# sergree/matchering

Hardware: NVIDIA H100
Metric: stereo 44.1kHz samples/sec (x real-time) (higher is better)
Workload: dtype f32

## Files before the change

### matchering_b200/csrc/common.cuh

```cuda
#pragma once

#ifndef MGB_EMULATE
#include <cuda_runtime.h>
#endif
#include <stdint.h>

#include "../../include/matchering_b200.h"

namespace mgb {

void set_error(const char* fmt, ...);
int cuda_status(const char* what);

#define MGB_REQUIRE(cond, code, ...)     \
    do {                                 \
        if (!(cond)) {                   \
            ::mgb::set_error(__VA_ARGS__); \
            return (code);               \
        }                                \
    } while (0)

#define MGB_TRY(expr)                 \
    do {                              \
        int mgb_rc_ = (expr);         \
        if (mgb_rc_ != MGB_OK) return mgb_rc_; \
    } while (0)

#ifdef MGB_EMULATE
#define MGB_DYN_SMEM(name) unsigned char* name = ::emul::dyn_smem()
template <typename... KA, typename... A>
inline int launch(const char* what, void (*kernel)(KA...), dim3 grid, dim3 block, size_t smem, cudaStream_t,
                  A... args) {
    (void)what;
    if (grid.x == 0 || grid.y == 0 || grid.z == 0) return MGB_OK;
    ::emul::launch(grid, block, smem, [&]() { kernel(static_cast<KA>(args)...); });
    return MGB_OK;
}
#else
#define MGB_DYN_SMEM(name) extern __shared__ __align__(128) unsigned char name[]
extern long long g_launch_count;
extern int g_profile;
void profile_mark(const char* what, cudaStream_t stream, bool begin);

template <typename... KA, typename... A>
inline int launch(const char* what, void (*kernel)(KA...), dim3 grid, dim3 block, size_t smem, cudaStream_t stream,
                  A... args) {
    if (grid.x == 0 || grid.y == 0 || grid.z == 0) return MGB_OK;
    g_launch_count++;
    if (smem > 48 * 1024) {
        static thread_local const void* done_kernel = nullptr;
        static thread_local size_t done_smem = 0;
        if (done_kernel != (const void*)kernel || done_smem < smem) {
            cudaError_t e = cudaFuncSetAttribute((const void*)kernel, cudaFuncAttributeMaxDynamicSharedMemorySize, (int)smem);
            if (e != cudaSuccess) {
                set_error("%s: cudaFuncSetAttribute(%zu B smem): %s", what, smem, cudaGetErrorString(e));
                return MGB_ERR_CUDA;
            }
            done_kernel = (const void*)kernel;
            done_smem = smem;
        }
    }
    if (g_profile) profile_mark(what, stream, true);
    kernel<<<grid, block, smem, stream>>>(static_cast<KA>(args)...);
    if (g_profile) profile_mark(what, stream, false);
    return cuda_status(what);
}
#endif

int num_sms();

template <typename T>
struct cpx {
    T x, y;
};
template <typename T>
__device__ __forceinline__ cpx<T> cmul(cpx<T> a, cpx<T> b) {
    return cpx<T>{a.x * b.x - a.y * b.y, a.x * b.y + a.y * b.x};
}
template <typename T>
__device__ __forceinline__ cpx<T> cadd(cpx<T> a, cpx<T> b) { return cpx<T>{a.x + b.x, a.y + b.y}; }
template <typename T>
__device__ __forceinline__ cpx<T> csub(cpx<T> a, cpx<T> b) { return cpx<T>{a.x - b.x, a.y - b.y}; }

__device__ __forceinline__ double warp_sum(double v) {
#pragma unroll
    for (int o = 16; o > 0; o >>= 1) v += __shfl_xor_sync(0xffffffffu, v, o);
    return v;
}
__device__ __forceinline__ float warp_max(float v) {
#pragma unroll
    for (int o = 16; o > 0; o >>= 1) v = fmaxf(v, __shfl_xor_sync(0xffffffffu, v, o));
    return v;
}

__device__ __forceinline__ double block_sum(double v, double* scratch) {
    const int lane = threadIdx.x & 31, warp = threadIdx.x >> 5, nwarps = (blockDim.x + 31) >> 5;
    v = warp_sum(v);
    __syncthreads();
    if (lane == 0) scratch[warp] = v;
    __syncthreads();
    if (warp == 0) {
        double t = (lane < nwarps) ? scratch[lane] : 0.0;
        t = warp_sum(t);
        if (lane == 0) scratch[0] = t;
    }
    __syncthreads();
    return scratch[0];
}
__device__ __forceinline__ float block_max(float v, float* scratch) {
    const int lane = threadIdx.x & 31, warp = threadIdx.x >> 5, nwarps = (blockDim.x + 31) >> 5;
    v = warp_max(v);
    __syncthreads();
    if (lane == 0) scratch[warp] = v;
    __syncthreads();
    if (warp == 0) {
        float t = (lane < nwarps) ? scratch[lane] : 0.0f;
        t = warp_max(t);
        if (lane == 0) scratch[0] = t;
    }
    __syncthreads();
    return scratch[0];
}

__device__ __forceinline__ unsigned warp_max_bits(unsigned v) {
#ifdef MGB_EMULATE
#pragma unroll
    for (int o = 16; o > 0; o >>= 1) {
        const unsigned other = __shfl_xor_sync(0xffffffffu, v, o);
        v = other > v ? other : v;
    }
    return v;
#else
    return __reduce_max_sync(0xffffffffu, v);
#endif
}
__device__ __forceinline__ void block_max2(float& a, float& b, unsigned* slot) {
    const unsigned ua = warp_max_bits(__float_as_uint(a)), ub = warp_max_bits(__float_as_uint(b));
    if ((threadIdx.x & 31) == 0) {
        atomicMax(&slot[0], ua);
        atomicMax(&slot[1], ub);
    }
    __syncthreads();
    a = __uint_as_float(slot[0]);
    b = __uint_as_float(slot[1]);
}

__device__ __forceinline__ float balance_factor(float large, float small) {
    if (!(small > 0.0f) || !(large > 0.0f)) return 1.0f;
    int e = (int)((__float_as_uint(large) >> 23) & 0xffu) - (int)((__float_as_uint(small) >> 23) & 0xffu);
    e = e < -60 ? -60 : (e > 60 ? 60 : e);
    return __uint_as_float((unsigned)(127 + e) << 23);
}

__device__ __forceinline__ float sqrt_approx(float x) {
#ifdef MGB_EMULATE
    return sqrtf(x);
#else
    float r;
    asm("sqrt.approx.ftz.f32 %0, %1;" : "=f"(r) : "f"(x));
    return r;
#endif
}

__device__ __forceinline__ void atomic_max_nonneg(float* addr, float v) {
    atomicMax(reinterpret_cast<int*>(addr), __float_as_int(v));
}
// ... 53 lines not shown
```

### matchering_b200/csrc/design.cu

```cuda
#include "fft.cuh"
#include "kernels.cuh"
#include "tail.cuh"

namespace mgb {

namespace {

constexpr int kDesignThreads = 512;
constexpr int kWarm = 48;
constexpr int kBatch = 16;
constexpr int kDesignBlocks = 4;

struct SplineTables {
    const double* hinv;
    const double* lu;
    const double* end;
};

__device__ void spline_moments(const double* __restrict__ y, int n, SplineTables t, double* __restrict__ z,
                               double* __restrict__ M) {
    const int m = n - 2;
    const double* fa = t.lu;
    const double* invden = t.lu + m;
    const double* cp = t.lu + 2 * m;
// ... 183 lines not shown
    double* M1 = m + HB;
    double* s = M1 + HB;
    double* mlog = s + HB;
    double* slog = mlog + NL;
    double* zz = slog + NL;
    double* M2 = zz + NL;

    spline_moments(m, HB, SplineTables{plan.d_sa_hinv, plan.d_sa_lu, plan.d_sa_end}, zz, M1);
    for (int j = tid; j < NL; j += nthr) mlog[j] = spline_eval(m, M1, plan.d_sa_eval_idx[j], plan.d_sa_eval_w + 4LL * j);
    __syncthreads();

    if (plan.lowess_it == 0) {
        const int k = plan.lowess_k;
        const int nfit = plan.lowess_nfit;
        for (int f = warp; f < nfit; f += 2 * nwarps) {
            const int f2 = min(f + nwarps, nfit - 1);
            const double* row_a = plan.d_lw_rows + (long long)plan.d_lw_row_idx[f] * k;
            const double* row_b = plan.d_lw_rows + (long long)plan.d_lw_row_idx[f2] * k;
            const double* ya = mlog + plan.d_lw_fit_left[f];
            const double* yb = mlog + plan.d_lw_fit_left[f2];
            double acc_a = 0.0, acc_b = 0.0;
            for (int j = lane; j < k; j += 32) {
                acc_a += row_a[j] * ya[j];
                acc_b += row_b[j] * yb[j];
            }
            acc_a = warp_sum(acc_a);
            acc_b = warp_sum(acc_b);
            if (lane == 0) {
                zz[f] = acc_a;
                zz[f2] = acc_b;
            }
        }
        __syncthreads();
        lowess_interpolate(plan, zz, slog);
    } else {
        double* resid_w = M2;
        for (int j = tid; j < NL; j += nthr) resid_w[j] = 1.0;
        __syncthreads();
        for (int pass = 0; pass <= plan.lowess_it; ++pass) {
            lowess_weighted_fits(plan, mlog, resid_w, zz);
            __syncthreads();
            lowess_interpolate(plan, zz, slog);
            if (pass < plan.lowess_it) lowess_residual_weights(mlog, slog, NL, zz, resid_w);
        }
    }

    spline_moments(slog, NL, SplineTables{plan.d_sb_hinv, plan.d_sb_lu, plan.d_sb_end}, zz, M2);
    for (int k = tid; k < HB; k += nthr) {
        double v = spline_eval(slog, M2, plan.d_sb_eval_idx[k], plan.d_sb_eval_w + 4LL * k);
        if (k == 0) v = 0.0;
        if (k == 1) v = m[1];
        s[k] = v;
    }
    __syncthreads();

}

struct DesignArgs {
    const float* spec_part_t;
    const float* spec_part_r;
    unsigned char* mask_t;
    unsigned char* mask_r;
    const float* absmax_t;
    float* target_peak;
    LevelsArgs levels;
    int div_t, slots_t, div_r, slots_r;
    long long frames_per_piece_t, frames_per_piece_r;
    const double* avg_override;
    double* scratch;
    long long stride;
    double* fir_out;
    float2* h_mid;
    float2* h_side;
    mgb_track_state* state;
    int s_ready;
    int ovs;
};

struct PrefetchList {
    const void* ptr[14];
    long long bytes[14];
    int count;
};

__device__ __forceinline__ void prefetch_l2(const void* p) {
#ifndef MGB_EMULATE
    asm volatile("prefetch.global.L2 [%0];" ::"l"(p));
#else
    (void)p;
#endif
}

constexpr int kMeanBins = 32, kMeanSlices = 32;

__global__ void __launch_bounds__(kMeanBins * kMeanSlices)
spectrum_mean_kernel(DesignArgs a, int n_lin, int fft_size, double eps, PrefetchList pf) {
    constexpr int BINS = kMeanBins, SLICES = kMeanSlices;
    __shared__ double part_t[SLICES][BINS + 1], part_r[SLICES][BINS + 1];
    MGB_DYN_SMEM(smem);
    unsigned char* mask_t = smem;
    unsigned char* mask_r = smem + a.div_t;
    {
        const long long gtid = ((long long)blockIdx.y * gridDim.x + blockIdx.x) * blockDim.x + threadIdx.x;
        const long long gsize = (long long)gridDim.x * gridDim.y * blockDim.x;
        for (int t = 0; t < pf.count; ++t)
            for (long long off = gtid * 128; off < pf.bytes[t]; off += gsize * 128)
                prefetch_l2(reinterpret_cast<const char*>(pf.ptr[t]) + off);
    }
    __shared__ LevelsResult lv_s;
    __shared__ unsigned peak_bits_s, target_peak_bits_s;
    double* piece_sum = reinterpret_cast<double*>(smem + ((a.div_t + a.div_r + 15) / 16) * 16);
    {
        const int lane = threadIdx.x & 31, warp = threadIdx.x >> 5, nwarps = blockDim.x >> 5;
        if (threadIdx.x == 0) peak_bits_s = target_peak_bits_s = 0u;
        __syncthreads();
        float pk = 0.0f;
        for (int i = threadIdx.x; i < a.div_r * a.slots_r + 1; i += blockDim.x) pk = fmaxf(pk, a.levels.absmax_r[i]);
        pk = warp_max_f(pk);
        if (lane == 0 && pk > 0.0f) atomicMax(&peak_bits_s, __float_as_uint(pk));
        if (blockIdx.x == 0 && blockIdx.y == 0) {
            float tpk = 0.0f;
            for (int i = threadIdx.x; i < a.div_t * a.slots_t + 1; i += blockDim.x) tpk = fmaxf(tpk, a.absmax_t[i]);
            tpk = warp_max_f(tpk);
            if (lane == 0 && tpk > 0.0f) atomicMax(&target_peak_bits_s, __float_as_uint(tpk));
        }
        for (int p = warp; p < a.div_t + a.div_r; p += nwarps) {
            const bool is_t = p < a.div_t;
            const double* part = is_t ? a.levels.sumsq_t + (long long)p * a.slots_t
                                      : a.levels.sumsq_r + (long long)(p - a.div_t) * a.slots_r;
            const int slots = is_t ? a.slots_t : a.slots_r;
            double sum = 0.0;
            for (int k = lane; k < slots; k += 32) sum += part[k];
            sum = warp_sum(sum);
            if (lane == 0) piece_sum[p] = sum;
        }
        __syncthreads();
        if (threadIdx.x < 32) {
            LevelsArgs folded = a.levels;
            folded.sumsq_t = piece_sum;
            folded.sumsq_r = piece_sum + a.div_t;
            folded.slots_t = folded.slots_r = 1;
            const float peak = __uint_as_float(peak_bits_s);
            folded.absmax_r = &peak;
            folded.div_r_items_override = 1;
            const LevelsResult mine = levels_compute_warp(folded, mask_t, mask_r);
            if (threadIdx.x == 0) lv_s = mine;
        }
    }
    __syncthreads();
    const LevelsResult lv = lv_s;
    if (blockIdx.x == 0 && blockIdx.y == 0) {
        if (threadIdx.x == 0) {
            levels_store(lv, a.state);
            a.state->conv_peak_bits = 0.0f;
            a.state->fir_peak_mid_bits = 0.0f;
            a.state->fir_peak_side_bits = 0.0f;
            a.state->conv_precise = 0;
            *a.target_peak = __uint_as_float(target_peak_bits_s);
        }
        for (int p = threadIdx.x; p < a.div_t; p += blockDim.x) a.mask_t[p] = mask_t[p];
        for (int p = threadIdx.x; p < a.div_r; p += blockDim.x) a.mask_r[p] = mask_r[p];
    }
    unsigned short* sel = reinterpret_cast<unsigned short*>(piece_sum + a.div_t + a.div_r);
    __shared__ int n_sel_s[2];
    int* piece_rank = reinterpret_cast<int*>(piece_sum);
    if (threadIdx.x < 32) {
        const int lane = threadIdx.x;
        for (int sig = 0; sig < 2; ++sig) {
            const unsigned char* mask = sig == 0 ? mask_t : mask_r;
            const int div = sig == 0 ? a.div_t : a.div_r;
            int* rank = piece_rank + (sig == 0 ? 0 : a.div_t);
            int count = 0;
            for (int base_p = 0; base_p < div; base_p += 32) {
                const int p = base_p + lane;
// ... 366 lines not shown
```

### matchering_b200/csrc/limiter.cu

```cuda
#include <math.h>
#include <string.h>

#include "limiter_scan.cuh"
#include "limiter_wide.cuh"

namespace mgb {

namespace {

constexpr int SPAN_EPT_MAX = kLimiterSpanEptMax;

__device__ __forceinline__ double scan_carry(double B, const ScanPow* t, double c0, double* scratch) {
    const int lane = threadIdx.x & 31, warp = threadIdx.x >> 5;
    double v = B;
#pragma unroll
    for (int d = 1; d < 32; d <<= 1) {
        const double up = __shfl_up_sync(0xffffffffu, v, d);
        if (lane >= d) v += t->ql[d] * up;
    }
    if (lane == 31) scratch[warp] = v;
    __syncthreads();
    double w = lane < NT / 32 ? scratch[lane] : 0.0;
#pragma unroll
    for (int d = 1; d < NT / 32; d <<= 1) {
        const double up = __shfl_up_sync(0xffffffffu, w, d);
        if (lane >= d) w += t->qw[d] * up;
    }
    const double warp_carry = __shfl_sync(0xffffffffu, w, (warp + 31) & 31);
    double prev = __shfl_up_sync(0xffffffffu, v, 1);
    if (lane == 0) prev = 0.0;
    return prev + t->ql[lane] * ((warp > 0 ? warp_carry : 0.0) + t->qw[warp] * c0);
}

__device__ __forceinline__ double scan_carry_rev(double B, const ScanPow* t, const double* c0, double* scratch) {
    const int lane = threadIdx.x & 31, warp = threadIdx.x >> 5;
    const int rl = 31 - lane, rw = NT / 32 - 1 - warp;
    double v = B;
#pragma unroll
    for (int d = 1; d < 32; d <<= 1) {
        const double up = __shfl_down_sync(0xffffffffu, v, d);
        if (rl >= d) v += t->ql[d] * up;
    }
    if (lane == 0) scratch[rw] = v;
    __syncthreads();
    double w = lane < NT / 32 ? scratch[lane] : 0.0;
#pragma unroll
    for (int d = 1; d < NT / 32; d <<= 1) {
        const double up = __shfl_up_sync(0xffffffffu, w, d);
        if (lane >= d) w += t->qw[d] * up;
    }
    const double warp_carry = __shfl_sync(0xffffffffu, w, (rw + 31) & 31);
    double prev = __shfl_down_sync(0xffffffffu, v, 1);
    if (rl == 0) prev = 0.0;
    return prev + t->ql[rl] * ((rw > 0 ? warp_carry : 0.0) + t->qw[rw] * (*c0));
}

struct LimiterGeom {
    int reach, hold, warm, left;
    int ept;
    int span;
    int filt;
    int publish_inclusive;
    int shared_core;
    int margin;
    int use_ticket;
};

__global__ void limiter_tables_kernel(mgb_limiter_params lp, int span_ept, unsigned char* tables) {
    const int i = threadIdx.x;
    ScanPow* att = reinterpret_cast<ScanPow*>(tables);
    {
        const double p = lp.attack_c;
        if (i < SPAN_EPT_MAX + 2) att->pe[i] = pow(p, (double)i);
        if (i < 33) att->ql[i] = pow(p, (double)(span_ept * i));
        if (i < 17) att->qw[i] = pow(p, (double)(span_ept * 32 * i));
        if (i < 33) att->pc[i] = pow(p, (double)LC * (double)i);
    }
    SectionTab<1>* sec = reinterpret_cast<SectionTab<1>*>(tables + sizeof(ScanPow));
    for (int f = 0; f < 2; ++f) {
        const double p = f == 0 ? -lp.hold_a[1] : -lp.release_a[1];
        SectionTab<1>* t = sec + f;
        if (i < CORE_EPT) t->pe[i][0] = pow(p, (double)(i + 1));
        if (i < 33) t->ql[i][0][0] = pow(p, (double)(CORE_EPT * i));
        if (i < 17) t->qw[i][0][0] = pow(p, (double)(CORE_EPT * 32 * i));
        if (i < 33) t->pc[i][0][0] = pow(p, (double)LC * (double)i);
        for (int j = i; j < kLookbackJumps; j += blockDim.x) t->pj[j][0][0] = pow(p, (double)LC * 32.0 * (double)j);
    }
}

template <int EPT, int NO, bool GAINS = false>
__global__ void __launch_bounds__(NT, (NO == 1 && EPT <= 17) ? 2 : 1)
limiter_kernel(mgb_limiter_params lp, LimiterGeom gm, const float2* __restrict__ in, float2* __restrict__ out,
               long long frames, const double* __restrict__ pre_gain, const double* __restrict__ post_gain,
               const int* __restrict__ engaged, int* __restrict__ ticket, LookbackWord* __restrict__ slots,
               const unsigned char* __restrict__ tables) {
    constexpr int HC = CORE_EPT + NO;
    constexpr int CAP = EPT * NT;
    MGB_DYN_SMEM(smem);
    double* Fd = reinterpret_cast<double*>(smem);
    float* Aenv = reinterpret_cast<float*>(smem) + CAP;
    float* G = reinterpret_cast<float*>(smem + (size_t)CAP * 8) + gm.margin;
    float* Wk = G + CAP + gm.margin;
    __shared__ float blockmax[NT];
    __shared__ ScanPow pw_att;
    __shared__ SectionTab<1> pw_sec[2];
    __shared__ double scratch_a[32 * NO], scratch_b[32 * NO];
    __shared__ double bcast[2 + 2 * NO];
    __shared__ int chunk_s;
    const ScanPow* pow_att = &pw_att;
    const SectionTab<NO>* sec_global = reinterpret_cast<const SectionTab<NO>*>(tables + sizeof(ScanPow));
    const SectionTab<NO>* tab_hold = NO == 1 ? reinterpret_cast<const SectionTab<NO>*>(&pw_sec[0]) : sec_global;
    const SectionTab<NO>* tab_rel = NO == 1 ? reinterpret_cast<const SectionTab<NO>*>(&pw_sec[1]) : sec_global + 1;

    const int tid = threadIdx.x;
    int chunk = blockIdx.x;
    if (gm.use_ticket) {
        if (tid == 0) chunk_s = atomicAdd(ticket, 1);
        __syncthreads();
        chunk = chunk_s;
    }
    const long long s0 = (long long)chunk * LC;
    const int core_n = (int)((s0 + LC < frames) ? LC : frames - s0);
    const int reach = gm.reach, hold = gm.hold, HL = gm.left, FL = gm.filt;
    const long long ga = s0 - HL - reach;
    const int cidx = HL + reach;
    const int vlo = ga < 0 ? (int)(-ga) : 0;
    const int vhi = (frames - ga < (long long)gm.span) ? (int)(frames - ga) : gm.span;
    const double thr = lp.threshold;

    float2 v[EPT];
    {
        const float2* base = in + ga;
#pragma unroll
        for (int k = 0; k < EPT; ++k) {
            const int i = tid + k * NT;
            v[k] = (i >= vlo && i < vhi) ? __ldg(base + i) : make_float2(0.0f, 0.0f);
        }
    }
    const double pre = pre_gain ? *pre_gain : 1.0;
    const double post = post_gain ? *post_gain : 1.0;
    const double scale = pre * post;
    const bool bypass = engaged && *engaged == 0;
    {
        const double* src = reinterpret_cast<const double*>(tables);
        double* dst = reinterpret_cast<double*>(&pw_att);
        for (int i = tid; i < (int)(sizeof(ScanPow) / sizeof(double)); i += NT) dst[i] = src[i];
        if (NO == 1) {
            src += sizeof(ScanPow) / sizeof(double);
            dst = reinterpret_cast<double*>(pw_sec);
            for (int i = tid; i < (int)(2 * sizeof(SectionTab<1>) / sizeof(double)); i += NT) dst[i] = src[i];
        }
    }
    if (bypass) {
        for (int k = tid; k < core_n; k += NT) {
            const float2 w = in[s0 + k];
            out[s0 + k] = make_float2((float)((double)w.x * pre * post), (float)((double)w.y * pre * post));
        }
        return;
    }
    for (int i = tid; i < gm.margin; i += NT) {
        G[-1 - i] = 0.0f;
        G[CAP + i] = 0.0f;
    }
#pragma unroll
    for (int k = 0; k < EPT; ++k) {
        const double a = (double)fmaxf(fabsf(v[k].x), fabsf(v[k].y)) * pre;
        const double over = a - thr;
        float g = 0.0f;
        if (over > 0.0) g = __fdiv_rn((float)over, (float)a);
        G[tid + k * NT] = g;
    }
    __syncthreads();

    float hc[HC];
    {
        float* PF = reinterpret_cast<float*>(smem);
        float* SF = Wk;
        float x[EPT];
        const int base = tid * EPT;
#pragma unroll
        for (int e = 0; e < EPT; ++e) x[e] = G[base + e];
        float run = 0.0f;
#pragma unroll
        for (int e = 0; e < EPT; ++e) {
            run = fmaxf(run, x[e]);
            PF[base + e] = run;
        }
        blockmax[tid] = run;
        run = 0.0f;
#pragma unroll
        for (int e = EPT - 1; e >= 0; --e) {
            run = fmaxf(run, x[e]);
            SF[base + e] = run;
        }
        __syncthreads();
        auto whole_blocks = [&](int a, int b) -> float {
            float m = 0.0f;
            for (int q = a; q <= b; ++q) m = fmaxf(m, blockmax[q]);
            return m;
        };
        auto window = [&](int l, int r, int br, float pr) -> float {
            const int bl = l / EPT;
            if (bl == br) {
                float m = 0.0f;
                for (int i = l; i <= r; ++i) m = fmaxf(m, G[i]);
                return m;
            }
            float m = fmaxf(SF[l], pr);
            if (br - bl > 1) m = fmaxf(m, whole_blocks(bl + 1, br - 1));
            return m;
        };
        auto gat = [&](int i) -> float { return G[i]; };
        if (gm.shared_core) {
            float la[EPT], rt[EPT];
#pragma unroll
            for (int e = 0; e < EPT - 1; ++e) {
                la[e] = gat(base - reach + e);
                rt[e + 1] = gat(base + reach + 1 + e);
            }
            la[EPT - 1] = rt[0] = 0.0f;
#pragma unroll
            for (int e = EPT - 2; e >= 0; --e) la[e] = fmaxf(la[e], la[e + 1]);
#pragma unroll
            for (int e = 1; e < EPT; ++e) rt[e] = fmaxf(rt[e], rt[e - 1]);
            const int r = min(base + reach, CAP - 1);
            const float core = window(max(base + EPT - 1 - reach, 0), r, r / EPT, PF[r]);
#pragma unroll
            for (int e = 0; e < EPT; ++e) Aenv[base + e] = fmaxf(core, fmaxf(la[e], rt[e]));
        } else {
#pragma unroll
            for (int e = 0; e < EPT; ++e) {
                const int i = base + e;
                const int r = min(i + reach, CAP - 1);
                Aenv[i] = window(max(i - reach, 0), r, r / EPT, PF[r]);
            }
        }
        const int bh = cidx + tid * CORE_EPT - NO;
        if (gm.shared_core) {
            float lh[HC], rh[HC];
#pragma unroll
            for (int e = 0; e < HC - 1; ++e) {
                lh[e] = gat(bh - reach - hold + 1 + e);
                rh[e + 1] = gat(bh + reach + 1 + e);
            }
            lh[HC - 1] = rh[0] = 0.0f;
#pragma unroll
            for (int e = HC - 2; e >= 0; --e) lh[e] = fmaxf(lh[e], lh[e + 1]);
#pragma unroll
            for (int e = 1; e < HC; ++e) rh[e] = fmaxf(rh[e], rh[e - 1]);
            const int r = min(bh + reach, CAP - 1);
            const float core = window(max(bh + HC - reach - hold, 0), r, r / EPT, PF[r]);
#pragma unroll
            for (int e = 0; e < HC; ++e) hc[e] = fmaxf(core, fmaxf(lh[e], rh[e]));
        } else {
#pragma unroll
            for (int e = 0; e < HC; ++e) {
                const int r = min(bh + e + reach, CAP - 1);
                hc[e] = window(max(bh + e - reach - hold + 1, 0), r, r / EPT, PF[r]);
            }
        }
#pragma unroll
        for (int e = 0; e < HC; ++e)
            if (bh + e < vlo) hc[e] = 0.0f;
    }

    LookbackWord* slot_hold = slots + (long long)chunk * (2 * NO);
    LookbackWord* slot_rel = slot_hold + NO;
    double hold_y[CORE_EPT];
    StVec<NO> hold_carry;
    float* Hown = Wk + tid * HC;
    {
#pragma unroll
        for (int e = 0; e < CORE_EPT; ++e) {
            double acc = lp.hold_b[0] * (double)hc[e + NO];
#pragma unroll
            for (int i = 1; i <= NO; ++i) acc += lp.hold_b[i] * (double)hc[e + NO - i];
#pragma unroll
            for (int i = 1; i <= NO; ++i)
                if (e - i >= 0) acc -= lp.hold_a[i] * hold_y[e - i];
            hold_y[e] = acc;
        }
        StVec<NO> end;
#pragma unroll
        for (int i = 0; i < NO; ++i) end.v[i] = hold_y[CORE_EPT - 1 - i];
        hold_carry = section_scan<NO>(end, tab_hold, scratch_a);
        if (tid == NT - 1) {
            st_addmul<NO>(end, tab_hold->ql[1], hold_carry);
            publish_state<NO>(slot_hold, end, 1);
        }
#pragma unroll
        for (int e = 0; e < HC; ++e) Hown[e] = hc[e];
    }

    const double c = lp.attack_c;
    const bool edge_l = vlo > reach, edge_r = vhi < reach + FL;
    if (edge_l || edge_r) {
        const int i0 = vlo, iL = vhi - 1;
        float fix[EPT];
#pragma unroll
        for (int k = 0; k < EPT; ++k) {
            const int i = tid + k * NT;
            fix[k] = Aenv[i];
            if (i < vlo) {
                const int d = (vlo - i < 6) ? vlo - i : 6;
                fix[k] = 2.0f * Aenv[i0] - Aenv[i0 + d];
            } else if (i >= vhi) {
                const int d = (i - iL < 6) ? i - iL : 6;
                fix[k] = 2.0f * Aenv[iL] - Aenv[iL - d];
            }
        }
        __syncthreads();
#pragma unroll
        for (int k = 0; k < EPT; ++k) Aenv[tid + k * NT] = fix[k];
        __syncthreads();
    }
    {
        double y[EPT];
        double acc = 0.0;
#pragma unroll
        for (int e = 0; e < EPT; ++e) {
            acc = (1.0 - c) * (double)Aenv[tid * EPT + e] + c * acc;
            y[e] = acc;
        }
        const double c0 = (double)Aenv[0];
        const double carry = scan_carry(acc, pow_att, c0, scratch_b);
#pragma unroll
        for (int e = 0; e < EPT; ++e) y[e] += pow_att->pe[e + 1] * carry;
        if (edge_r) {
            const int ilast = (int)(frames + 5 - ga);
            if (ilast < CAP - 1) {
#pragma unroll
                for (int e = 0; e < EPT; ++e)
                    if (tid * EPT + e == ilast) bcast[1] = y[e];
                __syncthreads();
                const double held = bcast[1];
#pragma unroll
                for (int e = 0; e < EPT; ++e)
                    if (tid * EPT + e > ilast) y[e] = held;
                __syncthreads();
            }
        }
        if (tid == NT - 1) bcast[1] = y[EPT - 1];
        acc = 0.0;
#pragma unroll
        for (int e = EPT - 1; e >= 0; --e) {
            acc = (1.0 - c) * y[e] + c * acc;
            y[e] = acc;
        }
        const double back = scan_carry_rev(acc, pow_att, &bcast[1], scratch_a);
#pragma unroll
        for (int e = 0; e < EPT; ++e) {
            const int i = tid * EPT + e;
            if (i >= cidx && i < cidx + LC) {
                const float att = (float)(y[e] + pow_att->pe[EPT - e] * back);
                G[i] = GAINS ? att : fmaxf(G[i], att);
            }
        }
    }

    if (tid < 32) {
        const StVec<NO> cin = lookback<NO>(slots, chunk, tab_hold);
        if (tid == 0) {
#pragma unroll
            for (int i = 0; i < NO; ++i) bcast[2 + i] = cin.v[i];
        }
    }
    __syncthreads();
    StVec<NO> hold_prev;
    {
        StVec<NO> cin;
#pragma unroll
        for (int i = 0; i < NO; ++i) cin.v[i] = bcast[2 + i];
        hold_prev = section_lead<NO>(tab_hold, cin);
#pragma unroll
        for (int i = 0; i < NO; ++i) hold_prev.v[i] += hold_carry.v[i];
#pragma unroll
        for (int e = 0; e < CORE_EPT; ++e)
#pragma unroll
            for (int i = 0; i < NO; ++i) hold_y[e] += tab_hold->pe[e][i] * hold_prev.v[i];
        if (tid == NT - 1 && gm.publish_inclusive) {
            StVec<NO> end;
#pragma unroll
            for (int i = 0; i < NO; ++i) end.v[i] = hold_y[CORE_EPT - 1 - i];
            publish_state<NO>(slot_hold, end, 2);
        }
    }

    {
        double rel_y[CORE_EPT];
        double win[HC];
#pragma unroll
        for (int i = 0; i < NO; ++i) win[i] = fmax((double)Hown[i], hold_prev.v[NO - 1 - i]);
#pragma unroll
        for (int e = 0; e < CORE_EPT; ++e) win[NO + e] = fmax((double)Hown[NO + e], hold_y[e]);
#pragma unroll
        for (int e = 0; e < CORE_EPT; ++e) {
            double acc = lp.release_b[0] * win[e + NO];
#pragma unroll
            for (int i = 1; i <= NO; ++i) acc += lp.release_b[i] * win[e + NO - i];
#pragma unroll
            for (int i = 1; i <= NO; ++i)
                if (e - i >= 0) acc -= lp.release_a[i] * rel_y[e - i];
            rel_y[e] = acc;
        }
        StVec<NO> end;
#pragma unroll
        for (int i = 0; i < NO; ++i) end.v[i] = rel_y[CORE_EPT - 1 - i];
        StVec<NO> rel_prev = section_scan<NO>(end, tab_rel, scratch_b);
        if (tid == NT - 1) {
            st_addmul<NO>(end, tab_rel->ql[1], rel_prev);
            publish_state<NO>(slot_rel, end, 1);
        }
        if (tid < 32) {
            const StVec<NO> cr = lookback<NO>(slots + NO, chunk, tab_rel);
            if (tid == 0) {
#pragma unroll
                for (int i = 0; i < NO; ++i) bcast[2 + NO + i] = cr.v[i];
            }
        }
        __syncthreads();
        {
            StVec<NO> cin;
#pragma unroll
            for (int i = 0; i < NO; ++i) cin.v[i] = bcast[2 + NO + i];
            const StVec<NO> lead = section_lead<NO>(tab_rel, cin);
#pragma unroll
            for (int i = 0; i < NO; ++i) rel_prev.v[i] += lead.v[i];
        }
#pragma unroll
        for (int e = 0; e < CORE_EPT; ++e) {
#pragma unroll
            for (int i = 0; i < NO; ++i) rel_y[e] += tab_rel->pe[e][i] * rel_prev.v[i];
            const int i = cidx + tid * CORE_EPT + e;
            const double g_rel = fmax(hold_y[e], rel_y[e]);
            Fd[tid * CORE_EPT + e] = GAINS ? g_rel : 1.0 - fmax((double)G[i], g_rel);
        }
        if (tid == NT - 1 && gm.publish_inclusive) {
#pragma unroll
            for (int i = 0; i < NO; ++i) end.v[i] = rel_y[CORE_EPT - 1 - i];
            publish_state<NO>(slot_rel, end, 2);
        }
    }
    if (GAINS) __syncthreads();
    else __syncwarp();

    {
        const int wbase = (tid >> 5) * (32 * CORE_EPT) + (tid & 31);
        float2 v[CORE_EPT];
#pragma unroll
        for (int q = 0; q < CORE_EPT; ++q) {
            const int k = wbase + q * 32;
            v[q] = k < core_n ? __ldg(in + s0 + k) : make_float2(0.0f, 0.0f);
        }
#pragma unroll
        for (int q = 0; q < CORE_EPT; ++q) {
            const int k = wbase + q * 32;
            if (k < core_n) {
                if (GAINS) {
                    out[s0 + k] = make_float2(G[cidx + k], (float)Fd[k]);
                } else {
                    const double gain = Fd[k] * scale;
                    out[s0 + k] = make_float2((float)((double)v[q].x * gain), (float)((double)v[q].y * gain));
                }
            }
        }
    }
}

__global__ void limiter_engaged_kernel(const float* peak_bits, const double* pre_gain, double threshold, int* engaged) {
    const double pre = pre_gain ? *pre_gain : 1.0;
    const double peak = (double)(*peak_bits) * pre;
    const double r = fmax(peak, threshold) / threshold;
    *engaged = (fabs(r - 1.0) <= 1e-8 + 1e-5 * 1.0) ? 0 : 1;
}

int limiter_order_capacity(const mgb_limiter_params& lp) {
    return (lp.hold_order <= 1 && lp.release_order <= 1) ? 1 : MGB_MAX_FILTER_ORDER;
}

}

int limiter_validate(const mgb_limiter_params& lp) {
    MGB_REQUIRE(lp.reach >= 1 && lp.hold >= 3 && lp.warmup >= 8, MGB_ERR_INVALID, "limiter: bad window sizes");
    MGB_REQUIRE(lp.hold_order >= 1 && lp.hold_order <= MGB_MAX_FILTER_ORDER && lp.release_order >= 1 &&
                    lp.release_order <= MGB_MAX_FILTER_ORDER,
                MGB_ERR_UNSUPPORTED, "limiter: hold / release filter orders %d / %d, kernels exist for 1..%d", lp.hold_order,
                lp.release_order, MGB_MAX_FILTER_ORDER);
    MGB_REQUIRE(lp.attack_c > 0.0 && lp.attack_c < 1.0, MGB_ERR_INVALID, "limiter: attack pole out of (0,1)");
    MGB_REQUIRE(lp.threshold > 0.0, MGB_ERR_INVALID, "limiter: threshold must be positive");
    return MGB_OK;
}

bool limiter_span_too_wide(const mgb_limiter_params& lp) {
    const long long no = limiter_order_capacity(lp), warm = lp.warmup, hold = lp.hold, reach = lp.reach;
    const long long left = warm > hold + no - 1 ? warm : hold + no - 1;
    const long long span = LC + left + warm + 2 * reach;
    return (span + NT - 1) / NT > SPAN_EPT_MAX;
}

namespace {

int limiter_geometry(const mgb_limiter_params& lp, LimiterGeom* g) {
    MGB_TRY(limiter_validate(lp));
    const int no = limiter_order_capacity(lp);
    g->reach = lp.reach;
    g->hold = lp.hold;
    g->warm = lp.warmup;
    g->left = lp.warmup > lp.hold + no - 1 ? lp.warmup : lp.hold + no - 1;
    g->filt = LC + g->left + g->warm;
    g->span = g->filt + 2 * g->reach;
    int ept = (g->span + NT - 1) / NT;
    if (!(ept & 1)) ept += 1;
    if (ept < 11) ept = 11;
    if (ept < CORE_EPT + no) ept = (CORE_EPT + no) | 1;
    g->ept = ept;
    g->publish_inclusive = g_lookback_inclusive;
    g->use_ticket = g_limiter_ticket;
    g->shared_core = (2 * lp.reach >= ept - 1 && 2 * lp.reach + lp.hold >= CORE_EPT + no) ? 1 : 0;
    g->margin = (lp.reach + lp.hold + ept + no + 3) / 4 * 4;
    MGB_REQUIRE(ept <= SPAN_EPT_MAX, MGB_ERR_UNSUPPORTED,
                "limiter: halo of %d samples exceeds the kernel's span", g->span - LC);
    return MGB_OK;
}

}

struct SectionPowers {
    long double A, B;
    int kind;
    long double r_log, theta, sin_theta;
    long double p1, p2;
    explicit SectionPowers(const double* a) {
        A = -(long double)a[1];
        B = (long double)a[2];
        if (a[2] == 0.0) {
            kind = 0;
            p1 = A;
            return;
        }
        const double hi = a[1] * a[1];
        const double lo = fma(a[1], a[1], -hi);
        const long double disc = ((long double)hi - 4.0L * B) + (long double)lo;
        if (disc < 0) {
            kind = 1;
            r_log = 0.5L * log1pl(B - 1.0L);
            theta = atan2l(sqrtl(-disc), A);
            sin_theta = sinl(theta);
        } else if (disc > 0) {
            kind = 2;
// ... 61 lines not shown
    return limiter_span_too_wide(lp) ? limiter_wide_plane_bytes(lp, frames) : 0;
}

int64_t limiter_tables_bytes() { return (int64_t)(sizeof(ScanPow) + 2 * sizeof(SectionTab<MGB_MAX_FILTER_ORDER>) + 255) / 256 * 256; }

int launch_limiter_tables(const mgb_limiter_params& lp, void* tables, cudaStream_t stream) {
    LimiterGeom g;
    MGB_TRY(limiter_validate(lp));
    if (limiter_span_too_wide(lp))
        g.ept = CORE_EPT;
    else
        MGB_TRY(limiter_geometry(lp, &g));
    if (limiter_order_capacity(lp) == 1)
        return launch("limiter_tables_kernel", limiter_tables_kernel, dim3(1), dim3(64), 0, stream, lp, g.ept,
                      (unsigned char*)tables);
    struct Block {
        ScanPow attack;
        SectionTab<2> section[2];
    } block;
    static_assert(sizeof(Block) == sizeof(ScanPow) + 2 * sizeof(SectionTab<2>), "table layout");
    fill_attack_tables(lp.attack_c, g.ept, &block.attack);
    fill_section_tables(lp.hold_a, &block.section[0]);
    fill_section_tables(lp.release_a, &block.section[1]);
#ifdef MGB_EMULATE
    (void)stream;
    memcpy(tables, &block, sizeof(block));
#else
    if (cudaMemcpyAsync(tables, &block, sizeof(block), cudaMemcpyHostToDevice, stream) != cudaSuccess) return cuda_status("limiter tables");
#endif
    return MGB_OK;
}

int launch_limiter(const mgb_limiter_params& lp, const float2* in, float2* out, int64_t frames, const double* pre_gain,
                   const double* post_gain, const int* engaged, int* ticket, void* lookback, void* wide_planes,
                   const void* tables, cudaStream_t stream, bool gains_only) {
    MGB_TRY(limiter_validate(lp));
    MGB_REQUIRE(frames > 6, MGB_ERR_INVALID, "limiter: the input must be longer than filtfilt's padlen (6)");
    MGB_REQUIRE(tables != nullptr, MGB_ERR_INVALID, "limiter: pole tables missing");
    if (limiter_span_too_wide(lp))
        return launch_limiter_wide(lp, limiter_order_capacity(lp), g_lookback_inclusive, in, out, frames, pre_gain, post_gain,
                                   engaged, lookback, wide_planes, tables, stream, gains_only);
    LimiterGeom g;
    MGB_TRY(limiter_geometry(lp, &g));
    const int64_t chunks = (frames + LC - 1) / LC;
    const size_t smem = (size_t)g.ept * NT * 16 + (size_t)g.margin * 8;
    const int no = limiter_order_capacity(lp);
    if (gains_only) {
        auto go = [&](auto kernel) {
            return launch("limiter_kernel", kernel, dim3((unsigned)chunks), dim3(NT), smem, stream, lp, g, in, out,
                          (long long)frames, pre_gain, post_gain, engaged, ticket, (LookbackWord*)lookback,
                          (const unsigned char*)tables);
        };
        if (no == 1 && g.ept == 11) return go(limiter_kernel<11, 1, true>);
        if (no == 1 && g.ept == 13) return go(limiter_kernel<13, 1, true>);
        if (no == MGB_MAX_FILTER_ORDER && g.ept == 11) return go(limiter_kernel<11, MGB_MAX_FILTER_ORDER, true>);
        set_error("limiter gains (test entry): no kernel for %d span samples per thread at order capacity %d", g.ept, no);
        return MGB_ERR_UNSUPPORTED;
    }
#define MGB_LIMITER_CASE(E)                                                                                           \
    case E:                                                                                                           \
        if (no == 1)                                                                                                  \
            return launch("limiter_kernel", limiter_kernel<E, 1>, dim3((unsigned)chunks), dim3(NT), smem, stream, lp, g, in, \
                          out, (long long)frames, pre_gain, post_gain, engaged, ticket, (LookbackWord*)lookback,     \
                          (const unsigned char*)tables);                                                             \
        return launch("limiter_kernel", limiter_kernel<E, MGB_MAX_FILTER_ORDER>, dim3((unsigned)chunks), dim3(NT), smem, \
                      stream, lp, g, in, out, (long long)frames, pre_gain, post_gain, engaged, ticket,               \
                      (LookbackWord*)lookback, (const unsigned char*)tables);
    switch (g.ept) {
        MGB_LIMITER_CASE(11)
        MGB_LIMITER_CASE(13)
        MGB_LIMITER_CASE(15)
        MGB_LIMITER_CASE(17)
        MGB_LIMITER_CASE(19)
        MGB_LIMITER_CASE(21)
        MGB_LIMITER_CASE(23)
        MGB_LIMITER_CASE(25)
        default: break;
    }
#undef MGB_LIMITER_CASE
    set_error("limiter: no kernel for %d span samples per thread", g.ept);
    return MGB_ERR_UNSUPPORTED;
}

int launch_limiter_engaged(const float* peak_bits, const double* pre_gain, double threshold, int* engaged,
                           cudaStream_t stream) {
    return launch("limiter_engaged_kernel", limiter_engaged_kernel, dim3(1), dim3(1), 0, stream, peak_bits, pre_gain,
                  threshold, engaged);
}

}
```

### matchering_b200/csrc/limiter_scan.cuh

```cuda
#pragma once
#include "kernels.cuh"

namespace mgb {

namespace {

constexpr int NT = kLimiterThreads;
constexpr int CORE_EPT = kLimiterCoreEpt;
constexpr int LC = kLimiterCore;

template <int N>
struct StVec {
    double v[N];
};
template <int N>
__device__ __forceinline__ StVec<N> st_zero() {
    StVec<N> z;
#pragma unroll
    for (int i = 0; i < N; ++i) z.v[i] = 0.0;
    return z;
}
template <int N>
__device__ __forceinline__ StVec<N> st_shfl_up(StVec<N> a, int d) {
#pragma unroll
    for (int i = 0; i < N; ++i) a.v[i] = __shfl_up_sync(0xffffffffu, a.v[i], d);
    return a;
}
template <int N>
__device__ __forceinline__ StVec<N> st_shfl(StVec<N> a, int src) {
#pragma unroll
    for (int i = 0; i < N; ++i) a.v[i] = __shfl_sync(0xffffffffu, a.v[i], src);
    return a;
}
template <int N>
__device__ __forceinline__ void st_addmul(StVec<N>& y, const double (*M)[N], const StVec<N>& x) {
#pragma unroll
    for (int r = 0; r < N; ++r)
#pragma unroll
        for (int c = 0; c < N; ++c) y.v[r] += M[r][c] * x.v[c];
}
template <int N>
__device__ __forceinline__ StVec<N> st_mul(const double (*M)[N], const StVec<N>& x) {
    StVec<N> y = st_zero<N>();
    st_addmul<N>(y, M, x);
    return y;
}

template <int N>
__device__ __forceinline__ StVec<N> section_scan(StVec<N> B, const SectionTab<N>* t, double* scratch) {
    const int lane = threadIdx.x & 31, warp = threadIdx.x >> 5;
    StVec<N> v = B;
#pragma unroll
    for (int d = 1; d < 32; d <<= 1) {
        const StVec<N> up = st_shfl_up<N>(v, d);
        if (lane >= d) st_addmul<N>(v, t->ql[d], up);
    }
    if (lane == 31) {
#pragma unroll
        for (int i = 0; i < N; ++i) scratch[warp * N + i] = v.v[i];
    }
    __syncthreads();
    StVec<N> w = st_zero<N>();
    if (lane < NT / 32) {
#pragma unroll
        for (int i = 0; i < N; ++i) w.v[i] = scratch[lane * N + i];
    }
#pragma unroll
    for (int d = 1; d < NT / 32; d <<= 1) {
        const StVec<N> up = st_shfl_up<N>(w, d);
        if (lane >= d) st_addmul<N>(w, t->qw[d], up);
    }
    StVec<N> warp_carry = st_shfl<N>(w, (warp + 31) & 31);
    if (warp == 0) warp_carry = st_zero<N>();
    StVec<N> prev = st_shfl_up<N>(v, 1);
    if (lane == 0) prev = st_zero<N>();
    st_addmul<N>(prev, t->ql[lane], warp_carry);
    return prev;
}

template <int N>
__device__ __forceinline__ StVec<N> section_lead(const SectionTab<N>* t, const StVec<N>& cin) {
    const int lane = threadIdx.x & 31, warp = threadIdx.x >> 5;
    return st_mul<N>(t->ql[lane], st_mul<N>(t->qw[warp], cin));
}

__device__ __forceinline__ void publish(LookbackWord* w, double v, int status) {
#ifdef MGB_EMULATE
    w->value = v;
    w->status = status;
#else
    asm volatile("st.global.cg.v2.u64 [%0], {%1, %2};" ::"l"(w), "l"(__double_as_longlong(v)), "l"((long long)status) : "memory");
#endif
}
__device__ __forceinline__ int poll(const LookbackWord* w, double* v) {
#ifdef MGB_EMULATE
    *v = w->value;
    return (int)w->status;
#else
    long long a, b;
    asm volatile("ld.global.cg.v2.u64 {%0, %1}, [%2];" : "=l"(a), "=l"(b) : "l"(w) : "memory");
    *v = __longlong_as_double(a);
    return (int)b;
#endif
}

template <int N>
__device__ __forceinline__ StVec<N> lookback(const LookbackWord* words , int chunk,
                                             const SectionTab<N>* t) {
    constexpr int STRIDE = 2 * N;
    const int lane = threadIdx.x & 31;
    if constexpr (N == 1) {
        double acc1 = 0.0, m1 = 1.0;
        for (int base = chunk - 1; base >= 0 && m1 > 1e-9; base -= 32) {
            const int j = base - lane;
            int st = 2;
            double val = 0.0;
            if (j >= 0) {
                const LookbackWord* w = words + (long long)j * STRIDE;
                while ((st = poll(w, &val)) == 0) __nanosleep(20);
            }
            const unsigned inclusive = __ballot_sync(0xffffffffu, st == 2);
            const int first = inclusive ? __ffs((int)inclusive) - 1 : 32;
            if (lane <= first) acc1 += m1 * t->pc[lane][0][0] * val;
            if (inclusive) break;
            m1 *= t->pc[32][0][0];
        }
        StVec<N> out;
        out.v[0] = warp_sum(acc1);
        return out;
    }
    StVec<N> acc = st_zero<N>();
    double mult[N][N];
    int jump = 0;
    for (int base = chunk - 1; base >= 0; base -= 32, ++jump) {
        if (N > 1 && jump < kLookbackJumps) {
#pragma unroll
            for (int r = 0; r < N; ++r)
#pragma unroll
                for (int c = 0; c < N; ++c) mult[r][c] = t->pj[jump][r][c];
        } else if (jump == 0) {
#pragma unroll
            for (int r = 0; r < N; ++r)
#pragma unroll
                for (int c = 0; c < N; ++c) mult[r][c] = r == c ? 1.0 : 0.0;
        } else {
            double next[N][N];
#pragma unroll
            for (int r = 0; r < N; ++r)
#pragma unroll
                for (int c = 0; c < N; ++c) {
                    double sum = 0.0;
#pragma unroll
                    for (int k = 0; k < N; ++k) sum += mult[r][k] * t->pc[32][k][c];
                    next[r][c] = sum;
                }
#pragma unroll
            for (int r = 0; r < N; ++r)
#pragma unroll
                for (int c = 0; c < N; ++c) mult[r][c] = next[r][c];
        }
// ... 42 lines not shown
```

Baseline: 559,600.

## Restructure limiter chunk kernel: merge scan barriers, sparse-table block max, prefetch input

Splits the hold and attack block scans into warp and block phases so both share one __syncthreads instead of two separate barrier sequences. Replaces the linear per-thread block-max loop with a warp-level sparse table plus prefix maxima, and keeps the attack envelope in registers instead of shared memory. The hold IIR zero-state is recomputed after the lookback rather than held in registers across it, and an L2 prefetch of the chunk's input is issued before the lookback wait. Optional globaltimer phase stamps are added behind a compile flag. The cost is extra recomputation and register pressure, plus more complex edge-handling code.

After: 569,400, median of 6. About the same (+1.8%).

```diff
diff --git a/matchering_b200/csrc/common.cuh b/matchering_b200/csrc/common.cuh
--- a/matchering_b200/csrc/common.cuh
+++ b/matchering_b200/csrc/common.cuh
@@ -82,6 +82,14 @@
 template <typename T>
 __device__ __forceinline__ cpx<T> csub(cpx<T> a, cpx<T> b) { return cpx<T>{a.x - b.x, a.y - b.y}; }
 
+__device__ __forceinline__ void prefetch_l2(const void* p) {
+#ifndef MGB_EMULATE
+    asm volatile("prefetch.global.L2 [%0];" ::"l"(p));
+#else
+    (void)p;
+#endif
+}
+
 __device__ __forceinline__ double warp_sum(double v) {
 #pragma unroll
     for (int o = 16; o > 0; o >>= 1) v += __shfl_xor_sync(0xffffffffu, v, o);
diff --git a/matchering_b200/csrc/design.cu b/matchering_b200/csrc/design.cu
--- a/matchering_b200/csrc/design.cu
+++ b/matchering_b200/csrc/design.cu
@@ -289,14 +289,6 @@
     long long bytes[14];
     int count;
 };
-
-__device__ __forceinline__ void prefetch_l2(const void* p) {
-#ifndef MGB_EMULATE
-    asm volatile("prefetch.global.L2 [%0];" ::"l"(p));
-#else
-    (void)p;
-#endif
-}
 
 constexpr int kMeanBins = 32, kMeanSlices = 32;
 
diff --git a/matchering_b200/csrc/limiter.cu b/matchering_b200/csrc/limiter.cu
--- a/matchering_b200/csrc/limiter.cu
+++ b/matchering_b200/csrc/limiter.cu
@@ -10,7 +10,24 @@
 
 constexpr int SPAN_EPT_MAX = kLimiterSpanEptMax;
 
-__device__ __forceinline__ double scan_carry(double B, const ScanPow* t, double c0, double* scratch) {
+#ifdef MGB_LIMITER_PHASE_CLOCKS
+constexpr int kPhaseStamps = 9, kPhaseChunksMax = 1 << 16;
+__device__ unsigned long long g_limiter_phase_clocks[kPhaseChunksMax * kPhaseStamps];
+#define MGB_PHASE(k)                                                                        \
+    do {                                                                                    \
+        if (tid == 0 && chunk < kPhaseChunksMax) {                                          \
+            unsigned long long t_;                                                          \
+            asm volatile("mov.u64 %0, %%globaltimer;" : "=l"(t_));                          \
+            g_limiter_phase_clocks[(long long)chunk * kPhaseStamps + (k)] = t_;              \
+        }                                                                                   \
+    } while (0)
+#else
+#define MGB_PHASE(k) \
+    do {             \
+    } while (0)
+#endif
+
+__device__ __forceinline__ double scan_carry_warp(double B, const ScanPow* t, double* scratch) {
     const int lane = threadIdx.x & 31, warp = threadIdx.x >> 5;
     double v = B;
 #pragma unroll
@@ -19,7 +36,10 @@
         if (lane >= d) v += t->ql[d] * up;
     }
     if (lane == 31) scratch[warp] = v;
-    __syncthreads();
+    return v;
+}
+__device__ __forceinline__ double scan_carry_block(double v, const ScanPow* t, double c0, const double* scratch) {
+    const int lane = threadIdx.x & 31, warp = threadIdx.x >> 5;
     double w = lane < NT / 32 ? scratch[lane] : 0.0;
 #pragma unroll
     for (int d = 1; d < NT / 32; d <<= 1) {
@@ -101,10 +121,9 @@
     float* Aenv = reinterpret_cast<float*>(smem) + CAP;
     float* G = reinterpret_cast<float*>(smem + (size_t)CAP * 8) + gm.margin;
     float* Wk = G + CAP + gm.margin;
-    __shared__ float blockmax[NT];
     __shared__ ScanPow pw_att;
     __shared__ SectionTab<1> pw_sec[2];
-    __shared__ double scratch_a[32 * NO], scratch_b[32 * NO];
+    __shared__ double scratch_a[32 * NO], scratch_b[32 * NO], scratch_c[32];
     __shared__ double bcast[2 + 2 * NO];
     __shared__ int chunk_s;
     const ScanPow* pow_att = &pw_att;
@@ -119,6 +138,7 @@
         __syncthreads();
         chunk = chunk_s;
     }
+    MGB_PHASE(0);
     const long long s0 = (long long)chunk * LC;
     const int core_n = (int)((s0 + LC < frames) ? LC : frames - s0);
     const int reach = gm.reach, hold = gm.hold, HL = gm.left, FL = gm.filt;
@@ -171,13 +191,17 @@
         G[tid + k * NT] = g;
     }
     __syncthreads();
+    MGB_PHASE(1);
 
     float hc[HC];
+    float aown[EPT];
     {
         float* PF = reinterpret_cast<float*>(smem);
         float* SF = Wk;
+        float* BT = Aenv;
+        float* BP = Aenv + 6 * NT;
         float x[EPT];
-        const int base = tid * EPT;
+        const int base = tid * EPT, lane = tid & 31;
 #pragma unroll
         for (int e = 0; e < EPT; ++e) x[e] = G[base + e];
         float run = 0.0f;
@@ -186,7 +210,23 @@
             run = fmaxf(run, x[e]);
             PF[base + e] = run;
         }
-        blockmax[tid] = run;
+        {
+            float m = run, p = run;
+            BT[tid] = m;
+#pragma unroll
+            for (int k = 1; k <= 5; ++k) {
+                const int d = 1 << (k - 1);
+                const float up = __shfl_down_sync(0xffffffffu, m, d);
+                if (lane + d < 32) m = fmaxf(m, up);
+                BT[k * NT + tid] = m;
+            }
+#pragma unroll
+            for (int d = 1; d < 32; d <<= 1) {
+                const float lo = __shfl_up_sync(0xffffffffu, p, d);
+                if (lane >= d) p = fmaxf(p, lo);
+            }
+            BP[tid] = p;
+        }
         run = 0.0f;
 #pragma unroll
         for (int e = EPT - 1; e >= 0; --e) {
@@ -195,8 +235,14 @@
         }
         __syncthreads();
         auto whole_blocks = [&](int a, int b) -> float {
-            float m = 0.0f;
-            for (int q = a; q <= b; ++q) m = fmaxf(m, blockmax[q]);
+            if (a > b) return 0.0f;
+            const int wa = a >> 5, wb = b >> 5;
+            if (wa == wb) {
+                const int k = 31 - __clz(b - a + 1);
+                return fmaxf(BT[k * NT + a], BT[k * NT + b - (1 << k) + 1]);
+            }
+            float m = fmaxf(BT[5 * NT + a], BP[b]);
+            for (int w = wa + 1; w < wb; ++w) m = fmaxf(m, BP[w * 32 + 31]);
             return m;
         };
         auto window = [&](int l, int r, int br, float pr) -> float {
@@ -226,13 +272,13 @@
             const int r = min(base + reach, CAP - 1);
             const float core = window(max(base + EPT - 1 - reach, 0), r, r / EPT, PF[r]);
 #pragma unroll
-            for (int e = 0; e < EPT; ++e) Aenv[base + e] = fmaxf(core, fmaxf(la[e], rt[e]));
+            for (int e = 0; e < EPT; ++e) aown[e] = fmaxf(core, fmaxf(la[e], rt[e]));
         } else {
 #pragma unroll
             for (int e = 0; e < EPT; ++e) {
                 const int i = base + e;
                 const int r = min(i + reach, CAP - 1);
-                Aenv[i] = window(max(i - reach, 0), r, r / EPT, PF[r]);
+                aown[e] = window(max(i - reach, 0), r, r / EPT, PF[r]);
             }
         }
         const int bh = cidx + tid * CORE_EPT - NO;
@@ -263,67 +309,81 @@
         for (int e = 0; e < HC; ++e)
             if (bh + e < vlo) hc[e] = 0.0f;
     }
+    MGB_PHASE(2);
 
     LookbackWord* slot_hold = slots + (long long)chunk * (2 * NO);
     LookbackWord* slot_rel = slot_hold + NO;
-    double hold_y[CORE_EPT];
-    StVec<NO> hold_carry;
     float* Hown = Wk + tid * HC;
-    {
+    auto hold_zero_state = [&](auto h, double(&y)[CORE_EPT]) {
 #pragma unroll
         for (int e = 0; e < CORE_EPT; ++e) {
-            double acc = lp.hold_b[0] * (double)hc[e + NO];
-#pragma unroll
-            for (int i = 1; i <= NO; ++i) acc += lp.hold_b[i] * (double)hc[e + NO - i];
+            double acc = lp.hold_b[0] * (double)h(e + NO);
+#pragma unroll
+            for (int i = 1; i <= NO; ++i) acc += lp.hold_b[i] * (double)h(e + NO - i);
 #pragma unroll
             for (int i = 1; i <= NO; ++i)
-                if (e - i >= 0) acc -= lp.hold_a[i] * hold_y[e - i];
-            hold_y[e] = acc;
-        }
-        StVec<NO> end;
-#pragma unroll
-        for (int i = 0; i < NO; ++i) end.v[i] = hold_y[CORE_EPT - 1 - i];
-        hold_carry = section_scan<NO>(end, tab_hold, scratch_a);
-        if (tid == NT - 1) {
-            st_addmul<NO>(end, tab_hold->ql[1], hold_carry);
-            publish_state<NO>(slot_hold, end, 1);
-        }
-#pragma unroll
-        for (int e = 0; e < HC; ++e) Hown[e] = hc[e];
+                if (e - i >= 0) acc -= lp.hold_a[i] * y[e - i];
+            y[e] = acc;
+        }
+    };
+    StVec<NO> hold_end;
+    {
+        double hold_y[CORE_EPT];
+        hold_zero_state([&](int e) { return hc[e]; }, hold_y);
+#pragma unroll
+        for (int i = 0; i < NO; ++i) hold_end.v[i] = hold_y[CORE_EPT - 1 - i];
     }
 
     const double c = lp.attack_c;
     const bool edge_l = vlo > reach, edge_r = vhi < reach + FL;
     if (edge_l || edge_r) {
+        __syncthreads();
+#pragma unroll
+        for (int e = 0; e < EPT; ++e) Aenv[tid * EPT + e] = aown[e];
+        __syncthreads();
         const int i0 = vlo, iL = vhi - 1;
-        float fix[EPT];
-#pragma unroll
-        for (int k = 0; k < EPT; ++k) {
-            const int i = tid + k * NT;
-            fix[k] = Aenv[i];
+#pragma unroll
+        for (int e = 0; e < EPT; ++e) {
+            const int i = tid * EPT + e;
             if (i < vlo) {
                 const int d = (vlo - i < 6) ? vlo - i : 6;
-                fix[k] = 2.0f * Aenv[i0] - Aenv[i0 + d];
+                aown[e] = 2.0f * Aenv[i0] - Aenv[i0 + d];
             } else if (i >= vhi) {
                 const int d = (i - iL < 6) ? i - iL : 6;
-                fix[k] = 2.0f * Aenv[iL] - Aenv[iL - d];
-            }
-        }
-        __syncthreads();
-#pragma unroll
-        for (int k = 0; k < EPT; ++k) Aenv[tid + k * NT] = fix[k];
-        __syncthreads();
-    }
+                aown[e] = 2.0f * Aenv[iL] - Aenv[iL - d];
+            }
+        }
+    }
+    if (tid == 0) bcast[0] = aown[0];
+    auto attack_forward = [&](double(&y)[EPT]) {
+        double acc = 0.0;
+#pragma unroll
+        for (int e = 0; e < EPT; ++e) {
+            acc = (1.0 - c) * (double)aown[e] + c * acc;
+            y[e] = acc;
+        }
+        return acc;
+    };
+    double att_end;
     {
         double y[EPT];
-        double acc = 0.0;
-#pragma unroll
-        for (int e = 0; e < EPT; ++e) {
-            acc = (1.0 - c) * (double)Aenv[tid * EPT + e] + c * acc;
-            y[e] = acc;
-        }
-        const double c0 = (double)Aenv[0];
-        const double carry = scan_carry(acc, pow_att, c0, scratch_b);
+        att_end = attack_forward(y);
+    }
+    const StVec<NO> hold_warp = section_scan_warp<NO>(hold_end, tab_hold, scratch_a);
+    const double att_warp = scan_carry_warp(att_end, pow_att, scratch_b);
+    __syncthreads();
+    const StVec<NO> hold_carry = section_scan_block<NO>(hold_warp, tab_hold, scratch_a);
+    if (tid == NT - 1) {
+        st_addmul<NO>(hold_end, tab_hold->ql[1], hold_carry);
+        publish_state<NO>(slot_hold, hold_end, 1);
+    }
+#pragma unroll
+    for (int e = 0; e < HC; ++e) Hown[e] = hc[e];
+    MGB_PHASE(3);
+    {
+        const double carry = scan_carry_block(att_warp, pow_att, bcast[0], scratch_b);
+        double y[EPT];
+        double acc = attack_forward(y);
 #pragma unroll
         for (int e = 0; e < EPT; ++e) y[e] += pow_att->pe[e + 1] * carry;
         if (edge_r) {
@@ -347,7 +407,7 @@
             acc = (1.0 - c) * y[e] + c * acc;
             y[e] = acc;
         }
-        const double back = scan_carry_rev(acc, pow_att, &bcast[1], scratch_a);
+        const double back = scan_carry_rev(acc, pow_att, &bcast[1], scratch_c);
 #pragma unroll
         for (int e = 0; e < EPT; ++e) {
             const int i = tid * EPT + e;
@@ -358,6 +418,12 @@
         }
     }
 
+    {
+        const unsigned long long first = reinterpret_cast<unsigned long long>(in + s0) & ~127ull;
+        const unsigned long long last = reinterpret_cast<unsigned long long>(in + s0 + core_n - 1) & ~127ull;
+        if (tid <= (int)((last - first) >> 7)) prefetch_l2(reinterpret_cast<const void*>(first + 128ull * tid));
+    }
+    MGB_PHASE(4);
     if (tid < 32) {
         const StVec<NO> cin = lookback<NO>(slots, chunk, tab_hold);
         if (tid == 0) {
@@ -366,8 +432,11 @@
         }
     }
     __syncthreads();
+    MGB_PHASE(5);
     StVec<NO> hold_prev;
-    {
+    double hold_y[CORE_EPT];
+    {
+        hold_zero_state([&](int e) { return Hown[e]; }, hold_y);
         StVec<NO> cin;
 #pragma unroll
         for (int i = 0; i < NO; ++i) cin.v[i] = bcast[2 + i];
@@ -411,6 +480,7 @@
             st_addmul<NO>(end, tab_rel->ql[1], rel_prev);
             publish_state<NO>(slot_rel, end, 1);
         }
+        MGB_PHASE(6);
         if (tid < 32) {
             const StVec<NO> cr = lookback<NO>(slots + NO, chunk, tab_rel);
             if (tid == 0) {
@@ -419,6 +489,7 @@
             }
         }
         __syncthreads();
+        MGB_PHASE(7);
         {
             StVec<NO> cin;
 #pragma unroll
@@ -465,6 +536,7 @@
             }
         }
     }
+    MGB_PHASE(8);
 }
 
 __global__ void limiter_engaged_kernel(const float* peak_bits, const double* pre_gain, double threshold, int* engaged) {
@@ -692,6 +764,17 @@
     return MGB_ERR_UNSUPPORTED;
 }
 
+#ifdef MGB_LIMITER_PHASE_CLOCKS
+}
+extern "C" int mgb_limiter_phase_clocks(unsigned long long* out, int chunks) {
+    if (chunks < 0 || chunks > mgb::kPhaseChunksMax) return MGB_ERR_INVALID;
+    const cudaError_t e = cudaMemcpyFromSymbol(out, mgb::g_limiter_phase_clocks,
+                                               (size_t)chunks * mgb::kPhaseStamps * sizeof(unsigned long long));
+    return e == cudaSuccess ? MGB_OK : MGB_ERR_CUDA;
+}
+namespace mgb {
+#endif
+
 int launch_limiter_engaged(const float* peak_bits, const double* pre_gain, double threshold, int* engaged,
                            cudaStream_t stream) {
     return launch("limiter_engaged_kernel", limiter_engaged_kernel, dim3(1), dim3(1), 0, stream, peak_bits, pre_gain,
diff --git a/matchering_b200/csrc/limiter_scan.cuh b/matchering_b200/csrc/limiter_scan.cuh
--- a/matchering_b200/csrc/limiter_scan.cuh
+++ b/matchering_b200/csrc/limiter_scan.cuh
@@ -47,7 +47,7 @@
 }
 
 template <int N>
-__device__ __forceinline__ StVec<N> section_scan(StVec<N> B, const SectionTab<N>* t, double* scratch) {
+__device__ __forceinline__ StVec<N> section_scan_warp(StVec<N> B, const SectionTab<N>* t, double* scratch) {
     const int lane = threadIdx.x & 31, warp = threadIdx.x >> 5;
     StVec<N> v = B;
 #pragma unroll
@@ -59,7 +59,11 @@
 #pragma unroll
         for (int i = 0; i < N; ++i) scratch[warp * N + i] = v.v[i];
     }
-    __syncthreads();
+    return v;
+}
+template <int N>
+__device__ __forceinline__ StVec<N> section_scan_block(const StVec<N>& v, const SectionTab<N>* t, const double* scratch) {
+    const int lane = threadIdx.x & 31, warp = threadIdx.x >> 5;
     StVec<N> w = st_zero<N>();
     if (lane < NT / 32) {
 #pragma unroll
@@ -76,6 +80,12 @@
     if (lane == 0) prev = st_zero<N>();
     st_addmul<N>(prev, t->ql[lane], warp_carry);
     return prev;
+}
+template <int N>
+__device__ __forceinline__ StVec<N> section_scan(StVec<N> B, const SectionTab<N>* t, double* scratch) {
+    const StVec<N> v = section_scan_warp<N>(B, t, scratch);
+    __syncthreads();
+    return section_scan_block<N>(v, t, scratch);
 }
 
 template <int N>
```
